# Tanveer81/ReVisionLLM

Hardware: AMD Instinct MI355X
Metric: video-segments/sec (whole node), stage-2 100-seg recursion, Vicuna-7B (higher is better)
Workload: dtype fp16

## Files before the change

### revisionllm_amd/csrc/engine.hip

```cpp
#include <string>
#include <unordered_map>
#include <vector>

#include "kernels.h"

struct Tensor {
    const void* p = nullptr;
    int dtype = 0;
    int64_t numel = 0;
};

struct AdapterLayer {
    const op16_t *w_in, *w_out, *w1, *w2;
    const float *b_in, *b_out, *b1, *b2, *ln1_w, *ln1_b, *ln2_w, *ln2_b;
};
struct LlmLayer {
    const op16_t *wqkv, *wo, *wgu, *wdown;
    const float *norm1, *norm2;
    const uint8_t *wqkv8 = nullptr, *wo8 = nullptr, *wgu8 = nullptr, *wdown8 = nullptr;
    const float *sqkv = nullptr, *so = nullptr, *sgu = nullptr, *sdown = nullptr;
    const uint8_t *wqkv8p = nullptr, *wo8p = nullptr, *wgu8p = nullptr, *wdown8p = nullptr;
    const op16_t *wqkv2 = nullptr, *wo2 = nullptr, *wgu2 = nullptr, *wdown2 = nullptr;
};

// ... 224 lines not shown
#define RV_TRY(expr)            \
    do {                        \
        int rc__ = (expr);      \
        if (rc__) return rc__;  \
    } while (0)

}

extern "C" int rv_ctx_create(const rv_config* cfg, rv_ctx** out) {
    RV_CHECK_ARG(out, "rv_ctx_create: null argument");
    if (!cfg) {
        rv_ctx* c = new rv_ctx();
        memset(&c->cfg, 0, sizeof(c->cfg));
        c->options_only = true;
        c->opt = g_default_opts;
        *out = c;
        return RV_OK;
    }
    RV_CHECK_ARG(cfg->hidden > 0 && cfg->heads > 0 && cfg->hidden % cfg->heads == 0, "rv_ctx_create: bad hidden/heads");
    RV_CHECK_ARG(cfg->hidden / cfg->heads == 128, "rv_ctx_create: LLM head dim must be 128 (got %d)", cfg->hidden / cfg->heads);
    RV_CHECK_ARG(cfg->hidden % 128 == 0 && cfg->inter % 128 == 0, "rv_ctx_create: hidden and inter must be multiples of 128");
    RV_CHECK_ARG(cfg->adapter_heads == 8 && (cfg->adapter_dim == 768 || (cfg->adapter_dim == 4096 && cfg->adapter_dim == cfg->hidden)),
                 "rv_ctx_create: the adapter is 768-d, or hidden-wide (4096) for the cross_attn ClipEncoder, with 8 heads");
    RV_CHECK_ARG(cfg->adapter_ff % 128 == 0 && cfg->adapter_layers >= 1, "rv_ctx_create: bad adapter ff/layers");
    rv_ctx* c = new rv_ctx();
    c->cfg = *cfg;
    c->opt = g_default_opts;
    *out = c;
    return RV_OK;
}

extern "C" void rv_ctx_destroy(rv_ctx* ctx) { delete ctx; }

namespace {
int* option_slot(RvOpts& o, const char* key) {
    const std::string k(key);
    if (k == "gemm_tile_variant") return &o.gemm_tile_variant;
    if (k == "gemm_cus") return &o.gemm_cus;
    if (k == "fp8_decode") return &o.fp8_decode;
    if (k == "fp8_prefill") return &o.fp8_prefill;
    if (k == "sample_variant") return &o.sample_variant;
    if (k == "gemm_arows") return &o.gemm_arows;
    if (k == "rows_fill") return &o.rows_fill;
    if (k == "rows_spread") return &o.rows_spread;
    if (k == "rows_persistent") return &o.rows_persistent;
    if (k == "rows_single") return &o.rows_single;
    if (k == "gemm_waves") return &o.gemm_waves;
    if (k == "gemm_mhalf") return &o.gemm_mhalf;
    if (k == "precision") return &o.precision;
    if (k == "lm_head_split") return &o.lm_head_split;
    if (k == "last_block_rows") return &o.last_block_rows;
    if (k == "adapter_stream16") return &o.adapter_stream16;
    if (k == "adapter_fold_t2v") return &o.adapter_fold_t2v;
    if (k == "attn_lds") return &o.attn_lds;
    if (k == "qkv_lds") return &o.qkv_lds;
    return nullptr;
}
}

unsigned int* rv_numeric_bound();

extern "C" int rv_ctx_set_option(rv_ctx* c, const char* key, int64_t value) {
    RV_CHECK_ARG(c && key, "rv_ctx_set_option: null argument");
    if (std::string(key) == "saturated") {
        RV_CHECK_ARG(value == 0, "rv_ctx_set_option: 'saturated' can only be reset to 0");
        if (unsigned int* p = rv_numeric_bound()) {
            if (hipDeviceSynchronize() != hipSuccess || hipMemset(p, 0, 16) != hipSuccess) {
                rv_set_error("rv_ctx_set_option: resetting the numeric status failed: %s", hipGetErrorString(hipGetLastError()));
                return RV_ERR_HIP;
            }
        }
        return RV_OK;
    }
    int* slot = option_slot(c->opt, key);
    RV_CHECK_ARG(slot, "rv_ctx_set_option: unknown option '%s'", key);
    const std::string k(key);
    if (k == "gemm_tile_variant") RV_CHECK_ARG(value >= 0 && value <= 6, "rv_ctx_set_option: gemm_tile_variant must be in [0, 6]");
    if (k == "gemm_waves") RV_CHECK_ARG(value == 4 || value == 8, "rv_ctx_set_option: gemm_waves must be 4 or 8");
    if (k == "gemm_cus") RV_CHECK_ARG(value >= 0 && value % 8 == 0, "rv_ctx_set_option: gemm_cus must be a non-negative multiple of 8");
    if (k == "precision") RV_CHECK_ARG(value == 0 || value == 1, "rv_ctx_set_option: precision must be 0 (bf16 operands) or 1 (parity: split operands)");
    *slot = (int)value;
    return RV_OK;
}

extern "C" int rv_ctx_get_option(const rv_ctx* c, const char* key, int64_t* value) {
    RV_CHECK_ARG(c && key && value, "rv_ctx_get_option: null argument");
    if (std::string(key) == "saturated") {
        *value = 0;
        if (unsigned int* p = rv_numeric_bound()) {
            unsigned int n = 0;
            if (hipDeviceSynchronize() != hipSuccess || hipMemcpy(&n, p, sizeof(n), hipMemcpyDeviceToHost) != hipSuccess) {
                rv_set_error("rv_ctx_get_option: reading the numeric status failed: %s", hipGetErrorString(hipGetLastError()));
                return RV_ERR_HIP;
            }
            *value = n;
        }
        return RV_OK;
    }
    const int* slot = option_slot(const_cast<rv_ctx*>(c)->opt, key);
    RV_CHECK_ARG(slot, "rv_ctx_get_option: unknown option '%s'", key);
    *value = *slot;
    return RV_OK;
}

extern "C" int rv_weights_bind(rv_ctx* c, const char* name, const void* dptr, int dtype, int64_t numel) {
    RV_CHECK_ARG(c && name && dptr && numel > 0, "rv_weights_bind: bad arguments");
// ... 11 lines not shown
    const int64_t d = c->cfg.adapter_dim, D = c->cfg.hidden;
    return rv_gemm_impl(x_bf16, d, c->proj_w, d, 1, c->proj_b, nullptr, 0, y, D, out_dtype, RV_ACT_NONE, rows, D, d, nullptr, 0, as_stream(stream));
}

extern "C" size_t rv_clip_encoder_ws_bytes(const rv_ctx* c, int32_t N, int32_t T, int32_t Nq, int32_t Lq) {
    if (!c || N <= 0 || T <= 0) return 0;
    return carve_clip(c, nullptr, 0, N, T, Nq, Lq).bytes;
}

extern "C" int rv_clip_encoder(rv_ctx* c, const void* x, const void* txt, const uint8_t* txt_mask, int32_t N, int32_t T,
                               int32_t Nq, int32_t Lq, int32_t feature, float* out, void* ws, size_t ws_bytes, void* stream) {
    RV_CHECK_ARG(c && x && out && ws, "rv_clip_encoder: null argument");
    RvOptScope scope(&c->opt);
    RV_CHECK_ARG(N > 0 && T > 0, "rv_clip_encoder: empty input N=%d T=%d", N, T);
    RV_CHECK_ARG(feature == RV_FEAT_CLS || feature == RV_FEAT_ALL, "rv_clip_encoder: feature must be CLS or ALL");
    RV_TRY(resolve_adapter(c));
    const bool text = c->cfg.adapter_text != 0;
    if (text) {
        RV_CHECK_ARG(txt && txt_mask && Nq > 0 && Lq > 0, "rv_clip_encoder: text features required (clip_adapter_text)");
        RV_CHECK_ARG(N % Nq == 0, "rv_clip_encoder: N=%d must be a multiple of Nq=%d", N, Nq);
    }
    hipStream_t st = as_stream(stream);
    const ClipWs w = carve_clip(c, ws, ws_bytes, N, T, text ? Nq : 0, text ? Lq : 0);
    if (w.bytes > ws_bytes) {
        rv_set_error("rv_clip_encoder: workspace %zu < required %zu", ws_bytes, w.bytes);
        return RV_ERR_WORKSPACE;
    }
    const int64_t d = c->cfg.adapter_dim, ff = c->cfg.adapter_ff, D = c->cfg.hidden;
    const int H = c->cfg.adapter_heads, dh = (int)(d / H);
    const float scale = 1.0f / sqrtf((float)dh);
    const int64_t R0 = (int64_t)N * T, R1 = (int64_t)N * (T + 1);

    const bool s16 = RV_OP_F16 != 0 && c->adp_proj_w != nullptr && c->opt.adapter_stream16 != 0 && (int64_t)N * T > 32;
    op16_t* xs16 = (op16_t*)w.x32;
    op16_t* ys16 = (op16_t*)w.y32;
    RV_TRY(k_copy_f32(c->cls_pos, w.pm, d, st));
    RV_TRY(k_sine_pos(w.pm + d, T, (int)d, st));

    if (text) {
        const int64_t RT = (int64_t)Nq * Lq;
        hipLaunchKernelGGL(invert_mask_kernel, dim3((unsigned)cdiv(RT, 256)), dim3(256), 0, st, txt_mask, w.pad, (int)RT);
        RV_CHECK_LAUNCH("invert_mask");
        float* v32 = w.x32;
        op16_t* vp16 = w.xp16;
        RV_TRY(k_frames_in(x, w.pm + d, s16 ? nullptr : v32, vp16, R0, T, (int)d, st));
        const op16_t* vres16 = (const op16_t*)x;
        for (size_t l = 0; l < c->t2v.size(); ++l) {
            const AdapterLayer& L = c->t2v[l];
            op16_t* q16 = w.qk16;
            RV_TRY(rv_gemm_impl(txt, d, L.w_in + d * d, d, 1, L.b_in + d, nullptr, 0, w.tk16, 2 * d, RV_OP16, RV_ACT_NONE, RT, 2 * d, d, w.sk, w.sk_bytes, st));
            const int LK = Lq <= 16 ? 16 : 32;
            const int64_t NK = (int64_t)H * LK, Rq = (int64_t)(N / Nq) * T;
            const bool fold = c->opt.adapter_fold_t2v != 0 && Lq <= 32 && dh <= 128 && NK % 64 == 0 && Rq > 32;
            if (fold) {
                float* S32 = (float*)w.qk16;
                op16_t* P16 = w.a16;
                RV_TRY(k_t2v_fold(L.w_in, L.b_in, L.w_out, w.tk16, w.tv16, 2 * d, Nq, Lq, LK, H, dh, scale, w.fa1, w.fc1, w.fa2, st));
                if (Nq > 1) {
                    RV_TRY(rv_gemm_grouped_impl(vp16, d, w.fa1, NK * d, w.fc1, NK, nullptr, 0, S32, NK, RV_F32, R0, NK, d, Rq, st));
                    RV_TRY(k_t2v_softmax(S32, w.pad, P16, R0, H, LK, Lq, Rq, st));
                    if (s16)
                        RV_TRY(rv_gemm_grouped_impl(P16, NK, w.fa2, NK * d, L.b_out, 0, (const float*)vres16, d, ys16, d, RV_OP16, R0, d, NK, Rq, st, 1));
                    else
                        RV_TRY(rv_gemm_grouped_impl(P16, NK, w.fa2, NK * d, L.b_out, 0, v32, d, w.y32, d, RV_F32, R0, d, NK, Rq, st));
                }
                for (int qi = 0; qi < Nq && Nq == 1; ++qi)
                    RV_TRY(rv_gemm_impl(vp16 + qi * Rq * d, d, w.fa1 + qi * NK * d, d, 1, w.fc1 + qi * NK, nullptr, 0, S32 + qi * Rq * NK, NK, RV_F32, RV_ACT_NONE, Rq, NK, d,
                                        w.sk, w.sk_bytes, st));
                if (Nq == 1) RV_TRY(k_t2v_softmax(S32, w.pad, P16, R0, H, LK, Lq, Rq, st));
                for (int qi = 0; qi < Nq && Nq == 1; ++qi) {
                    const int64_t r0 = qi * Rq;
                    if (s16)
                        RV_TRY(rv_gemm_impl(P16 + r0 * NK, NK, w.fa2 + qi * NK * d, NK, 1, L.b_out, (const float*)(vres16 + r0 * d), d, ys16 + r0 * d, d, RV_OP16, RV_ACT_NONE, Rq, d,
                                            NK, w.sk, w.sk_bytes, st, nullptr, 1));
                    else
                        RV_TRY(rv_gemm_impl(P16 + r0 * NK, NK, w.fa2 + qi * NK * d, NK, 1, L.b_out, v32 + r0 * d, d, w.y32 + r0 * d, d, RV_F32, RV_ACT_NONE, Rq, d, NK, w.sk,
                                            w.sk_bytes, st));
                }
            } else {
                RV_TRY(rv_gemm_impl(vp16, d, L.w_in, d, 1, L.b_in, nullptr, 0, q16, d, RV_OP16, RV_ACT_NONE, R0, d, d, w.sk, w.sk_bytes, st));
                RV_TRY(k_transpose_v(w.tv16, 2 * d, w.tvt16, Nq, Lq, w.Lqpad, H, dh, st));
                AttnArgs a{q16, d, (int64_t)T * d, w.tk16, 2 * d, (int64_t)Lq * 2 * d, dh, w.tvt16, (int64_t)d * w.Lqpad, (int64_t)dh * w.Lqpad,
                           w.Lqpad, w.a16, d, (int64_t)T * d, w.pad, N, H, dh, T, Lq, 0, 0, N / Nq, scale};
                RV_TRY(k_attention(a, st));
            }
            if (s16) {
                if (!fold)
                    RV_TRY(rv_gemm_impl(w.a16, d, L.w_out, d, 1, L.b_out, (const float*)vres16, d, ys16, d, RV_OP16, RV_ACT_NONE, R0, d, d, w.sk, w.sk_bytes, st, nullptr, 1));
                RV_TRY(k_layernorm(nullptr, L.ln1_w, L.ln1_b, nullptr, w.x16, nullptr, nullptr, 0, R0, (int)d, st, 0, ys16));
                RV_TRY(rv_gemm_impl(w.x16, d, L.w1, d, 1, L.b1, nullptr, 0, w.h16, ff, RV_OP16, RV_ACT_RELU, R0, ff, d, w.sk, w.sk_bytes, st));
                RV_TRY(rv_gemm_impl(w.h16, ff, L.w2, ff, 1, L.b2, (const float*)ys16, d, ys16, d, RV_OP16, RV_ACT_NONE, R0, d, ff, w.sk, w.sk_bytes, st, nullptr, 1));
                if (l + 1 < c->t2v.size()) {
                    RV_TRY(k_layernorm(nullptr, L.ln2_w, L.ln2_b, nullptr, xs16, vp16, w.pm + d, T, R0, (int)d, st, 0, ys16));
                    vres16 = xs16;
                } else {
                    RV_TRY(k_layernorm(nullptr, L.ln2_w, L.ln2_b, nullptr, w.x16, w.xp16, w.pm + d, T, R0, (int)d, st, T, ys16));
                    RV_TRY(k_cls_rows(c->cls_token, w.pm, nullptr, w.x16, w.xp16, N, T, (int)d, st));
                }
                continue;
            }
            if (!fold)
                RV_TRY(rv_gemm_impl(w.a16, d, L.w_out, d, 1, L.b_out, v32, d, w.y32, d, RV_F32, RV_ACT_NONE, R0, d, d, w.sk, w.sk_bytes, st));
            RV_TRY(k_layernorm(w.y32, L.ln1_w, L.ln1_b, nullptr, w.x16, nullptr, nullptr, 0, R0, (int)d, st));
            RV_TRY(rv_gemm_impl(w.x16, d, L.w1, d, 1, L.b1, nullptr, 0, w.h16, ff, RV_OP16, RV_ACT_RELU, R0, ff, d, w.sk, w.sk_bytes, st));
            RV_TRY(rv_gemm_impl(w.h16, ff, L.w2, ff, 1, L.b2, w.y32, d, w.y32, d, RV_F32, RV_ACT_NONE, R0, d, ff, w.sk, w.sk_bytes, st));
            if (l + 1 < c->t2v.size()) {
                RV_TRY(k_layernorm(w.y32, L.ln2_w, L.ln2_b, v32, nullptr, vp16, w.pm + d, T, R0, (int)d, st));
            } else {
                RV_TRY(k_layernorm(w.y32, L.ln2_w, L.ln2_b, w.x32, w.x16, w.xp16, w.pm + d, T, R0, (int)d, st, T));
                RV_TRY(k_cls_rows(c->cls_token, w.pm, w.x32, w.x16, w.xp16, N, T, (int)d, st));
            }
        }
    } else {
        RV_TRY(k_build_x(x, nullptr, c->cls_token, w.pm, s16 ? nullptr : w.x32, w.x16, w.xp16, N, T, (int)d, st));
    }

    for (size_t l = 0; l < c->enc.size(); ++l) {
        const AdapterLayer& L = c->enc[l];
        if (feature == RV_FEAT_CLS && l + 1 == c->enc.size() && N > 16 && T >= 3) {
            const int64_t sx = (int64_t)(T + 1) * d;
            op16_t* kk16 = w.qk16;
            op16_t* qc16 = w.h16;
            float* y0 = w.y32;
            float* y1 = w.y32 + (int64_t)N * d;
            float* y2 = w.y32 + (int64_t)2 * N * d;
            RV_TRY(rv_gemm_impl(w.xp16, d, L.w_in + d * d, d, 1, L.b_in + d, nullptr, 0, kk16, d, RV_OP16, RV_ACT_NONE, R1, d, d, w.sk, w.sk_bytes, st));
            RV_TRY(rv_gemm_impl(w.xp16, sx, L.w_in, d, 1, L.b_in, nullptr, 0, qc16, d, RV_OP16, RV_ACT_NONE, N, d, d, w.sk, w.sk_bytes, st, nullptr, 0, 1));
            RV_TRY(rv_gemm_impl(w.x16, d, L.w_in + 2 * d * d, d, 1, L.b_in + 2 * d, nullptr, 0, w.vv16, d, RV_OP16, RV_ACT_NONE, R1, d, d, w.sk, w.sk_bytes, st));
            RV_TRY(k_transpose_v(w.vv16, d, w.vt16, N, T + 1, w.Lpad, H, dh, st));
            AttnArgs a{qc16, d, d, kk16, d, (int64_t)(T + 1) * d, dh, w.vt16, (int64_t)d * w.Lpad, (int64_t)dh * w.Lpad, w.Lpad, w.a16, d, d,
                       nullptr, N, H, dh, 1, T + 1, 0, 0, 1, scale, 1};
            RV_TRY(k_attention(a, st));
            const float* cls_res = w.x32;
            int64_t cls_ld = sx;
            if (s16) {
                float* y3 = w.y32 + (int64_t)3 * N * d;
                RV_TRY(k_rows_to_f32(w.x16, sx, y3, N, (int)d, st));
                cls_res = y3;
                cls_ld = d;
            }
            RV_TRY(rv_gemm_impl(w.a16, d, L.w_out, d, 1, L.b_out, cls_res, cls_ld, y0, d, RV_F32, RV_ACT_NONE, N, d, d, w.sk, w.sk_bytes, st, nullptr, 0, 1));
            RV_TRY(k_layernorm(y0, L.ln1_w, L.ln1_b, y1, w.x16, nullptr, nullptr, 0, N, (int)d, st, 0, nullptr, s16 ? 3 : 0));
// ... 533 lines not shown
```

### revisionllm_amd/csrc/kernels.h

```cpp
#pragma once
#include "common.h"

struct RvOpts {
    int gemm_tile_variant = 2;
    int gemm_cus = 0;
    int fp8_decode = 1;
    int fp8_prefill = 1;
    int sample_variant = 1;
    int gemm_arows = 1;
    int gemm_waves = 8;
    int gemm_mhalf = 2;
    int rows_single = 1;
    int rows_persistent = 1;
    int rows_spread = 0;
    int rows_fill = 240;
    int lm_head_split = 1;
    int last_block_rows = 1;
    int adapter_stream16 = 1;
    int adapter_fold_t2v = 1;
    int attn_lds = 1;
    int qkv_lds = 1;
    int precision = 0;
};
extern const RvOpts g_default_opts;
const RvOpts& rv_cur_opts();
struct RvOptScope {
    const RvOpts* prev;
    explicit RvOptScope(const RvOpts* o);
    ~RvOptScope();
};
const RvOpts* rv_ctx_opts(const rv_ctx* c);

struct GemvNorm {
    const float* in_sumsq = nullptr;
    int in_nblk = 0;
    float inv_d = 0.f, eps = 0.f;
    void* xw_out = nullptr;
    const float* w_next = nullptr;
    float* out_sumsq = nullptr;
    const float* w_scale = nullptr;
    int x_packed = 0;
    int out_packed = 0;
    float* planes = nullptr;
    int* arrive = nullptr;
};
__host__ __device__ __forceinline__ int64_t rv_xp_index(int r, int k, int mbp) {
    return ((((int64_t)(k >> 5) * mbp + (r >> 4)) * 64 + (r & 15) + 16 * ((k >> 3) & 3)) * 8) + (k & 7);
}
constexpr int RV_ROWS_COUNTERS = 2048;
constexpr int RV_ROWS_MAX = 144;
constexpr int RV_XP_MAX_BLOCKS = 9;
__host__ __device__ __forceinline__ int rv_xp_blocks(int64_t rows) { return rows <= 32 ? 2 : rows <= 64 ? 4 : rows <= 80 ? 5 : rows <= 128 ? 8 : 9; }

constexpr int RV_MAX_PREFILL_GROUPS = 8;
__host__ __device__ __forceinline__ int64_t rv_vt_index(int d, int pos) { return ((int64_t)(pos >> 3) * 128 + d) * 8 + (pos & 7); }
struct alignas(32) QkvGroup {
    int base, B, S, P0, row, pad_[3];
};
struct QkvRope {
    const float* cs = nullptr;
    void* q16 = nullptr;
    void* kc = nullptr;
    void* vtc = nullptr;
    int B = 0, S = 0, P0 = 0, pos0 = 0, cs_pos0 = 0, H = 0, Smax = 0;
    const int* row_pos = nullptr;
    int G = 1, Mg = 0;
    int grow[RV_MAX_PREFILL_GROUPS] = {0, 0, 0, 0, 0, 0, 0, 0};
    int q_ld = 0, q_lo = 0;
    int ng = 0;
    const QkvGroup* gt = nullptr;
};
static __device__ __forceinline__ QkvGroup qkv_rope_group(const QkvRope& q, int& m) {
// ... 91 lines not shown
}
static __device__ __forceinline__ void qkv_rope_store(const QkvRope& q, int m, int n, f32x4 v) {
    qkv_rope_store(q, m, n, v, qkv_rope_coeffs(q, m, n));
}

int gemm_qkv_rope(const void* A, int64_t lda, const void* Wp, int64_t M, int64_t D, const QkvRope& r, const GemvNorm* norm,
                  void* ws, size_t ws_bytes, hipStream_t st, int w_layout = 1, int64_t Kdim = 0);

int rv_gemm_impl(const void* A, int64_t lda, const void* W, int64_t ldw, int w_layout, const float* bias,
                 const float* residual, int64_t ldr, void* C, int64_t ldc, int out_dtype, int act, int64_t M, int64_t N,
                 int64_t K, void* ws, size_t ws_bytes, hipStream_t st, const GemvNorm* norm = nullptr, int res16 = 0, int no_stream = 0);
struct GemmGroups {
    int rows = 0, tiles = 0;
    int64_t w_stride = 0, bias_stride = 0;
};
int rv_gemm_grouped_impl(const void* A, int64_t lda, const void* Wp, int64_t w_stride, const float* bias, int64_t bias_stride, const float* residual, int64_t ldr, void* C,
                         int64_t ldc, int out_dtype, int64_t M, int64_t N, int64_t K, int64_t rows_per_group, hipStream_t st, int res16 = 0);
int gemv_blocks(int act, int64_t N);
int gemm_rows(const op16_t* X, const op16_t* W, const float* bias, const float* res, int64_t ldr, void* C, int64_t ldc, int out_dtype, int act,
              int M, int N, int K, hipStream_t st, const GemvNorm& nrm, const QkvRope* qr, int w_layout = 1);
size_t gemm_rows_ws_bytes();
bool gemm_arows_supported(int w_layout, int act, int64_t M, int64_t N, int64_t K);
int gemm_arows_launch(const void* A, int64_t lda, const void* Wp, const float* bias, const float* res, int64_t ldr, void* C, int64_t ldc,
                      int out_dtype, int act, int64_t M, int64_t N, int64_t K, hipStream_t st);
bool gemm_pp_supported(int w_layout, int64_t M, int64_t N, int64_t K);
bool gemm_pp_sk_supported(int w_layout, int64_t M, int64_t N, int64_t K);
int gemm_pp_sk_plan(int64_t M, int64_t N, int64_t K, bool gated);
bool gemm_pp_sk_profitable(int64_t M, int64_t N, int64_t K);
bool gemm_pp_dp_profitable(int64_t M, int64_t N, int64_t K);
int gemm_pp_dp_plan(int64_t M, int64_t N, int64_t K, bool gated);
size_t gemm_pp_ws_bytes();
bool gemm_pp_fp8_supported(int64_t M, int64_t N, int64_t K, bool gated, bool rope);
int gemm_pp_fp8(const void* A8, int64_t lda, const float* sa, const void* W8p, const float* sw, const float* res, int64_t ldr, void* C,
                int64_t ldc, int out_dtype, int act, int64_t M, int64_t N, int64_t K, const QkvRope* r, void* ws, hipStream_t st);
int gemm_pp_launch(const void* A, int64_t lda, const void* Wp, const float* bias, const float* res, int64_t ldr, void* C,
                   int64_t ldc, int out_dtype, int act, int64_t M, int64_t N, int64_t K, void* ws, hipStream_t st);
int gemm_pp_qkv_rope(const void* A, int64_t lda, const void* Wp, int64_t M, int64_t N, int64_t K, const QkvRope& r, void* ws,
                     hipStream_t st);
int k_layernorm(const float* x, const float* w, const float* b, float* y32, void* y16, void* yp16, const float* pos,
                int64_t period, int64_t rows, int d, hipStream_t st, int64_t gap = 0, const void* x_op16 = nullptr, int rnd = 0);
int k_rmsnorm_quant(const float* x, int64_t x_row_stride, const float* w, void* q8, float* scale, int64_t rows, int d, float eps,
                    hipStream_t st);
int k_quant_rows_fp8(const void* x16, int64_t ldx, void* q8, int64_t ldq, float* scale, int64_t rows, int K, hipStream_t st);
int k_rmsnorm(const float* x, int64_t x_row_stride, const float* w, void* y16, int64_t rows, int d, float eps, hipStream_t st,
              int out_packed = 0, const int* row_idx = nullptr);
int k_rmsnorm_split(const float* x, int64_t x_row_stride, const float* w, void* y16, int64_t rows, int d, float eps, hipStream_t st, int out_packed = 0,
                    const int* row_idx = nullptr);
int k_split_bf16(const float* x, int64_t ldx, void* y16, int64_t rows, int n, hipStream_t st);
int k_qkv_rope_split(const float* qkv32, int64_t ld, const QkvRope& qr, int64_t M, int64_t D, hipStream_t st);
int k_gather_last_rows(const void* a16, const float* h, const int* idx, int64_t rows, int Mg, int P0, int B, int S, void* a_out, float* h_out, int D, hipStream_t st);
int k_t2v_fold(const void* wq_p, const float* bq, const void* wo_p, const void* tk16, const void* tv16, int64_t ld, int Nq, int Lq, int LK, int H, int dh, float scale,
               void* A1p, float* c1, void* A2p, hipStream_t st);
int k_t2v_softmax(const float* S, const uint8_t* pad, void* P16, int64_t rows, int H, int LK, int Lq, int64_t rows_per_query, hipStream_t st);
int k_sine_pos(float* pos, int T, int d, hipStream_t st);
int k_frames_in(const void* x16, const float* pos, float* v32, void* vp16, int64_t rows, int T, int d, hipStream_t st);
int k_build_x(const void* src16, const float* src32, const float* cls, const float* pm, float* x32, void* x16, void* xp16,
              int64_t N, int T, int d, hipStream_t st);
int k_copy_f32(const float* src, float* dst, int64_t n, hipStream_t st);
int k_rows_to_f32(const void* src16, int64_t ld, float* dst, int64_t rows, int d, hipStream_t st);
int k_cls_rows(const float* cls, const float* pm, float* x32, void* x16, void* xp16, int64_t N, int T, int d, hipStream_t st);
int k_transpose_v(const void* v, int64_t ld, void* vt, int64_t Nb, int L, int Lpad, int H, int dh, hipStream_t st);
int k_rope_table(float* cs, int S, int pos0, int dh, float theta, hipStream_t st);
int k_rope_table_rows(float* cs, const int* row_pos, int rows, int dh, float theta, hipStream_t st);
int k_splice_embed(const int32_t* map, const void* embed, const float* video, float* h, int64_t rows, int D, hipStream_t st);

struct AttnArgs {
    const void* q; int64_t q_rs, q_bs;
    const void* k; int64_t k_rs, k_bs, k_hs;
    const void* vt; int64_t vt_bs, vt_hs, vt_ds;
    void* out; int64_t o_rs, o_bs;
    const uint8_t* key_pad;
    int B, H, dh, Lq, Lk, causal, q_pos0, kv_div;
    float scale;
    int no_split = 0;
    const int* row_pos = nullptr;
    int out_packed = 0;
    int64_t vt_ks = 8;
    int64_t out_lo = 0;
    int64_t q_lo = 0;
    const int* row_share = nullptr;
};
int k_attention(const AttnArgs& a, hipStream_t st);
struct AttnGroups {
    int G = 1;
    int64_t q_off[RV_MAX_PREFILL_GROUPS] = {0, 0, 0, 0, 0, 0, 0, 0};
    int64_t o_off[RV_MAX_PREFILL_GROUPS] = {0, 0, 0, 0, 0, 0, 0, 0};
    int64_t kv_off[RV_MAX_PREFILL_GROUPS] = {0, 0, 0, 0, 0, 0, 0, 0};
};
int k_attention_pair(const AttnArgs& a, const AttnArgs& b, hipStream_t st, const AttnGroups* groups = nullptr);
int k_attention_groups(const AttnArgs& a, hipStream_t st, const AttnGroups& groups);
struct AttnMixed {
    int G = 0, problems = 0;
    int first[RV_MAX_PREFILL_GROUPS] = {};
    QkvGroup gt[RV_MAX_PREFILL_GROUPS] = {};
};
int k_attention_mixed(const AttnArgs& a, const AttnMixed& mx, hipStream_t st);
int k_mixed_tables(const AttnMixed& mx, QkvGroup* gt, int* last_rows, hipStream_t st);
```

### revisionllm_amd/csrc/rowops.hip

```cpp
#include "common.h"
#include "kernels.h"

namespace {

template <int NV>
__global__ __launch_bounds__(256) void layernorm_kernel(const float* __restrict__ x, const float* __restrict__ w,
                                                        const float* __restrict__ b, float* __restrict__ y32,
                                                        op16_t* __restrict__ y16, op16_t* __restrict__ yp16,
                                                        const float* __restrict__ pos, int64_t period, int64_t rows, int64_t gap,
                                                        const op16_t* __restrict__ x16in, int rnd) {
    constexpr int D = NV * 256;
    const int lane = threadIdx.x & 63;
    const int64_t row = (int64_t)blockIdx.x * 4 + (threadIdx.x >> 6);
    if (row >= rows) return;
    const float* xr = x + row * D;
    const int64_t orow = gap > 0 ? row + row / gap + 1 : row;
    f32x4 v[NV];
    float s = 0.f;
#pragma unroll
    for (int i = 0; i < NV; ++i) {
        v[i] = x16in ? op16x4_to_f32(*(const u32x2*)(x16in + row * D + i * 256 + lane * 4)) : *(const f32x4*)(xr + i * 256 + lane * 4);
        if (rnd & 1) v[i] = op16x4_to_f32(pack_op16x4(f32x4{v[i][0], v[i][1], v[i][2], v[i][3]}));
        s += v[i][0] + v[i][1] + v[i][2] + v[i][3];
    }
// ... 360 lines not shown
                    const f32x4 kk = *(const f32x4*)&rr[j][t];
#pragma unroll
                    for (int e = 0; e < 4; ++e) acc += kk[e] * w[t + e];
                }
                const int hj = h * LK + j;
                if (which) A2p[(int64_t)q * NK * d + rv_wp_index(k, hj, NK)] = f32_to_op16(acc);
                else A1p[(int64_t)q * NK * d + rv_wp_index(hj, k, d)] = f32_to_op16(acc * mul);
            }
        }
        if (blockIdx.x == 0 && threadIdx.x < 64) {
            for (int j = 0; j < LK; ++j) {
                float c = 0.f;
                for (int t = threadIdx.x; t < DH; t += 64) c += rr[j][t] * bq[h * DH + t];
                c = wave_sum(c);
                if (threadIdx.x == 0) c1[(int64_t)q * NK + h * LK + j] = c * scale;
            }
        }
    }
}

template <int LK>
__global__ __launch_bounds__(256) void t2v_softmax_kernel(const float* __restrict__ S, const uint8_t* __restrict__ pad, op16_t* __restrict__ P, int64_t rows, int H, int Lq,
                                                          int64_t rows_per_query) {
    const int64_t i = (int64_t)blockIdx.x * 256 + threadIdx.x;
    if (i >= rows * H) return;
    const int64_t r = i / H;
    const uint8_t* pq = pad + (r / rows_per_query) * Lq;
    unsigned valid = 0u;
    for (int j = 0; j < Lq; ++j) valid |= (pq[j] == 0 ? 1u : 0u) << j;
    const f32x4* s4 = (const f32x4*)(S + i * LK);
    f32x4 v[LK / 4];
    float mx = -INFINITY;
#pragma unroll
    for (int c = 0; c < LK / 4; ++c) {
        v[c] = s4[c];
#pragma unroll
        for (int e = 0; e < 4; ++e) {
            if (!((valid >> (c * 4 + e)) & 1u)) v[c][e] = -INFINITY;
            mx = fmaxf(mx, v[c][e]);
        }
    }
    float z = 0.f;
#pragma unroll
    for (int c = 0; c < LK / 4; ++c)
#pragma unroll
        for (int e = 0; e < 4; ++e) {
            v[c][e] = mx == -INFINITY ? 0.f : __expf(v[c][e] - mx);
            z += v[c][e];
        }
    const float iz = z > 0.f ? 1.0f / z : 0.f;
    u32x2* p2 = (u32x2*)(P + i * LK);
#pragma unroll
    for (int c = 0; c < LK / 4; ++c) p2[c] = pack_op16x4(f32x4{v[c][0] * iz, v[c][1] * iz, v[c][2] * iz, v[c][3] * iz});
}

__global__ void rope_table_kernel(float2* __restrict__ cs, int S, int pos0, int dh, float theta) {
    const int i = blockIdx.x * blockDim.x + threadIdx.x;
    const int half = dh / 2;
    if (i >= S * half) return;
    const int s = i / half, j = i % half;
    const float inv = 1.0f / powf(theta, (float)(2 * j) / (float)dh);
    const float ang = (float)(pos0 + s) * inv;
    cs[i] = make_float2(cosf(ang), sinf(ang));
}

__global__ void rope_table_rows_kernel(float2* __restrict__ cs, const int* __restrict__ row_pos, int rows, int dh, float theta) {
    const int i = blockIdx.x * blockDim.x + threadIdx.x;
    const int half = dh / 2;
    if (i >= rows * half) return;
    const int s = i / half, j = i % half;
    const int pos = row_pos[s] > 0 ? row_pos[s] : 0;
    const float inv = 1.0f / powf(theta, (float)(2 * j) / (float)dh);
    const float ang = (float)pos * inv;
    cs[i] = make_float2(cosf(ang), sinf(ang));
}

__global__ __launch_bounds__(256) void splice_embed_kernel(const int32_t* __restrict__ map, const op16_t* __restrict__ embed,
                                                           const float* __restrict__ video, float* __restrict__ h, int D) {
    const int64_t r = blockIdx.x;
    const int src = map[r];
    float* o = h + r * D;
    if (src >= 0) {
        const op16_t* e = embed + (int64_t)src * D;
        for (int c = threadIdx.x * 4; c < D; c += 1024) {
            const u32x2 raw = *(const u32x2*)(e + c);
            *(f32x4*)(o + c) = op16x4_to_f32(raw);
        }
    } else {
        const float* v = video + (int64_t)(-(src + 1)) * D;
        for (int c = threadIdx.x * 4; c < D; c += 1024) *(f32x4*)(o + c) = *(const f32x4*)(v + c);
    }
}

}

int k_layernorm(const float* x, const float* w, const float* b, float* y32, void* y16, void* yp16, const float* pos,
                int64_t period, int64_t rows, int d, hipStream_t st, int64_t gap, const void* x_op16, int rnd) {
    RV_CHECK_ARG((x || x_op16) && w && b && rows >= 0, "layernorm: bad arguments");
    RV_CHECK_ARG(!yp16 || (pos && period > 0), "layernorm: y_pos needs pos table and period");
    if (rows == 0) return RV_OK;
    const unsigned blocks = (unsigned)cdiv(rows, 4);
    if (d == 768)
        hipLaunchKernelGGL(layernorm_kernel<3>, dim3(blocks), dim3(256), 0, st, x, w, b, y32, (op16_t*)y16, (op16_t*)yp16, pos, period, rows, gap, (const op16_t*)x_op16, rnd);
    else if (d == 4096)
        hipLaunchKernelGGL(layernorm_kernel<16>, dim3(blocks), dim3(256), 0, st, x, w, b, y32, (op16_t*)y16, (op16_t*)yp16, pos, period, rows, gap, (const op16_t*)x_op16, rnd);
    else if (d == 1024)
// ... 115 lines not shown
    if (dh == 96)
        hipLaunchKernelGGL(transpose_v_kernel<96>, grid, dim3(256), 0, st, (const op16_t*)v, ld, (op16_t*)vt, L, Lpad, H);
    else if (dh == 128)
        hipLaunchKernelGGL(transpose_v_kernel<128>, grid, dim3(256), 0, st, (const op16_t*)v, ld, (op16_t*)vt, L, Lpad, H);
    else if (dh == 512)
        hipLaunchKernelGGL(transpose_v_kernel<512>, dim3(grid.x, grid.y * 4, grid.z), dim3(256), 0, st, (const op16_t*)v, ld, (op16_t*)vt, L, Lpad, H);
    else {
        rv_set_error("transpose_v: head dim %d unsupported", dh);
        return RV_ERR_ARG;
    }
    RV_CHECK_LAUNCH("transpose_v");
    return RV_OK;
}

int k_gather_last_rows(const void* a16, const float* h, const int* idx, int64_t rows, int Mg, int P0, int B, int S, void* a_out, float* h_out, int D, hipStream_t st) {
    RV_CHECK_ARG(a16 && h && a_out && h_out && rows > 0 && D % 4 == 0, "gather_last_rows: bad arguments");
    hipLaunchKernelGGL(gather_last_rows_kernel, dim3((unsigned)rows), dim3(256), 0, st, (const op16_t*)a16, h, idx, Mg, P0, B, S, (op16_t*)a_out, h_out, D);
    RV_CHECK_LAUNCH("gather_last_rows");
    return RV_OK;
}

int k_t2v_fold(const void* wq_p, const float* bq, const void* wo_p, const void* tk16, const void* tv16, int64_t ld, int Nq, int Lq, int LK, int H, int dh, float scale,
               void* A1p, float* c1, void* A2p, hipStream_t st) {
    const int d = H * dh;
    RV_CHECK_ARG(wq_p && bq && wo_p && tk16 && tv16 && A1p && c1 && A2p && ld >= d && Nq > 0 && Lq > 0 && Lq <= LK && (LK == 16 || LK == 32) && dh <= 128 && d % 32 == 0,
                 "t2v_fold: bad arguments");
#define RV_FOLD_REG(DH_, LK_)                                                                                                                                  \
    hipLaunchKernelGGL((t2v_fold_reg_kernel<DH_, LK_>), dim3((unsigned)(2 * cdiv(d, 256)), (unsigned)H, (unsigned)cdiv(Nq, qpw)), dim3(256), 0, st, (const op16_t*)wq_p, bq, \
                       (const op16_t*)wo_p, (const op16_t*)tk16, (const op16_t*)tv16, ld, Lq, H, d, scale, (op16_t*)A1p, c1, (op16_t*)A2p, Nq, qpw)
    const bool reg = Nq >= 3;
    const int qpw = (int)cdiv((int64_t)Nq * 2 * cdiv(d, 256) * H, 1024);
    if (reg && dh == 96 && LK == 16) RV_FOLD_REG(96, 16);
    else if (reg && dh == 96 && LK == 32) RV_FOLD_REG(96, 32);
    else if (reg && dh == 64 && LK == 16) RV_FOLD_REG(64, 16);
    else if (reg && dh == 64 && LK == 32) RV_FOLD_REG(64, 32);
    else
        hipLaunchKernelGGL(t2v_fold_kernel, dim3((unsigned)cdiv(d, 256), (unsigned)(H * LK), (unsigned)Nq), dim3(256), 0, st, (const op16_t*)wq_p, bq, (const op16_t*)wo_p,
                           (const op16_t*)tk16, (const op16_t*)tv16, ld, Lq, LK, H, dh, d, scale, (op16_t*)A1p, c1, (op16_t*)A2p);
#undef RV_FOLD_REG
    RV_CHECK_LAUNCH("t2v_fold");
    return RV_OK;
}

int k_t2v_softmax(const float* S, const uint8_t* pad, void* P16, int64_t rows, int H, int LK, int Lq, int64_t rows_per_query, hipStream_t st) {
    RV_CHECK_ARG(S && pad && P16 && rows > 0 && (LK == 16 || LK == 32) && Lq <= LK && rows_per_query > 0, "t2v_softmax: bad arguments");
    if (LK == 16)
        hipLaunchKernelGGL(t2v_softmax_kernel<16>, dim3((unsigned)cdiv(rows * H, 256)), dim3(256), 0, st, S, pad, (op16_t*)P16, rows, H, Lq, rows_per_query);
    else
        hipLaunchKernelGGL(t2v_softmax_kernel<32>, dim3((unsigned)cdiv(rows * H, 256)), dim3(256), 0, st, S, pad, (op16_t*)P16, rows, H, Lq, rows_per_query);
    RV_CHECK_LAUNCH("t2v_softmax");
    return RV_OK;
}

int k_rope_table(float* cs, int S, int pos0, int dh, float theta, hipStream_t st) {
    hipLaunchKernelGGL(rope_table_kernel, dim3((unsigned)cdiv((int64_t)S * (dh / 2), 256)), dim3(256), 0, st, (float2*)cs, S, pos0, dh, theta);
    RV_CHECK_LAUNCH("rope_table");
    return RV_OK;
}

int k_rope_table_rows(float* cs, const int* row_pos, int rows, int dh, float theta, hipStream_t st) {
    hipLaunchKernelGGL(rope_table_rows_kernel, dim3((unsigned)cdiv((int64_t)rows * (dh / 2), 256)), dim3(256), 0, st, (float2*)cs, row_pos, rows, dh, theta);
    RV_CHECK_LAUNCH("rope_table_rows");
    return RV_OK;
}

int k_splice_embed(const int32_t* map, const void* embed, const float* video, float* h, int64_t rows, int D, hipStream_t st) {
    hipLaunchKernelGGL(splice_embed_kernel, dim3((unsigned)rows), dim3(256), 0, st, map, (const op16_t*)embed, video, h, D);
    RV_CHECK_LAUNCH("splice_embed");
    return RV_OK;
}

extern "C" int rv_layernorm(const float* x, const float* w, const float* b, float* y_f32, void* y_bf16, void* y_pos_bf16,
                            const float* pos, int64_t period, int64_t rows, int32_t d, void* stream) {
    return k_layernorm(x, w, b, y_f32, y_bf16, y_pos_bf16, pos, period, rows, d, as_stream(stream));
}
extern "C" int rv_rmsnorm(const float* x, const float* w, void* y_bf16, int64_t rows, int32_t d, float eps, void* stream) {
    return k_rmsnorm(x, d, w, y_bf16, rows, d, eps, as_stream(stream));
}
extern "C" int rv_rmsnorm_quant_fp8(const float* x, const float* w, void* q8, float* scale, int64_t rows, int32_t d, float eps, void* stream) {
    RV_CHECK_ARG(x && w && q8 && scale, "rv_rmsnorm_quant_fp8: null argument");
    return k_rmsnorm_quant(x, d, w, q8, scale, rows, d, eps, as_stream(stream));
}
extern "C" int rv_sine_pos(float* pos, int32_t T, int32_t d, void* stream) { return k_sine_pos(pos, T, d, as_stream(stream)); }
```

### revisionllm_amd/hip.py

```python
import ctypes as C
import os

import torch

_HERE = os.path.dirname(os.path.abspath(__file__))
LIB_PATHS = {"f16": os.environ.get("REVISION_HIP_LIB") or os.path.join(_HERE, "librevision_hip.so"),
             "bf16": os.environ.get("REVISION_HIP_LIB_BF16") or os.path.join(_HERE, "librevision_hip_bf16.so")}
LIB_PATH = LIB_PATHS["f16"]
OP_DTYPES = {"f16": torch.float16, "bf16": torch.bfloat16}

RV_F32, RV_BF16, RV_I32, RV_I64, RV_U8, RV_F16 = 0, 1, 2, 3, 4, 5
RV_ACT_NONE, RV_ACT_RELU, RV_ACT_SILU_MUL, RV_ACT_QUICK_GELU = 0, 1, 2, 3
RV_FEAT_CLS, RV_FEAT_ALL = 0, 2
TOPK_CAP = 64

_DT = {torch.float32: RV_F32, torch.bfloat16: RV_BF16, torch.float16: RV_F16, torch.int32: RV_I32, torch.int64: RV_I64, torch.uint8: RV_U8}


class RvConfig(C.Structure):
    _fields_ = [("hidden", C.c_int32), ("inter", C.c_int32), ("layers", C.c_int32), ("heads", C.c_int32),
                ("vocab", C.c_int32), ("rms_eps", C.c_float), ("rope_theta", C.c_float), ("adapter_dim", C.c_int32),
                ("adapter_heads", C.c_int32), ("adapter_ff", C.c_int32), ("adapter_layers", C.c_int32),
                ("adapter_text", C.c_int32)]

# ... 147 lines not shown
            raise HipLibraryError(
                f"{path} not found: build it with `python -m revisionllm_amd.build` (hipcc, gfx950). "
                "revisionllm_amd has no CPU fallback.")
        try:
            h = C.CDLL(path)
        except OSError as e:
            raise HipLibraryError(f"cannot load {path}: {e}") from e
        for name, (res, args) in SIGNATURES.items():
            fn = getattr(h, name)
            fn.restype, fn.argtypes = res, args
        if h.rv_operand_dtype() != _DT[OP_DTYPES[f]]:
            raise HipLibraryError(f"{path} is not the {f} build of the library (rv_operand_dtype() = {h.rv_operand_dtype()})")
        _libs[f] = h
    return h


_numeric = {}


def numeric_status(f=None, device=None):
    f = flavour_of(f)
    dev = torch.device("cuda", torch.cuda.current_device()) if device is None else torch.device(device)
    if dev.index is None:
        dev = torch.device("cuda", torch.cuda.current_device())
    key = (f, dev.index)
    t = _numeric.get(key)
    if t is None:
        t = torch.zeros(4, dtype=torch.int32, device=dev)
        with torch.cuda.device(dev):
            torch.cuda.synchronize(dev)
            check(lib(f).rv_numeric_status_bind(C.c_void_p(t.data_ptr())), "rv_numeric_status_bind")
        _numeric[key] = t
    return t


def last_error():
    buf = C.create_string_buffer(512)
    msgs = []
    for h in _libs.values():
        h.rv_last_error(buf, 512)
        if buf.value:
            msgs.append(buf.value.decode())
    return " | ".join(msgs)


def check(rc, what):
    if rc != 0:
        msgs = last_error().split(" | ")
        name = what.split("(")[0]
        mine = [m for m in msgs if name in m]
        raise HipLibraryError(f"{what} failed (status {rc}): {' | '.join(mine or msgs)}")


OPTION_KEYS = ("gemm_tile_variant", "gemm_cus", "gemm_arows", "fp8_decode", "fp8_prefill", "sample_variant", "rows_fill", "rows_spread", "rows_persistent", "rows_single", "gemm_waves", "gemm_mhalf", "precision", "lm_head_split", "last_block_rows", "adapter_stream16", "adapter_fold_t2v", "attn_lds", "qkv_lds")


class Options:

    def __init__(self, flavour=None, **kw):
        self.flavour = flavour_of(flavour)
        self.lib = lib(self.flavour)
        self._ctx = C.c_void_p()
        check(self.lib.rv_ctx_create(None, C.byref(self._ctx)), "rv_ctx_create(options)")
        for k, v in kw.items():
            self.set(k, v)

    def set(self, key, value):
        check(self.lib.rv_ctx_set_option(self._ctx, key.encode(), int(value)), f"rv_ctx_set_option({key})")
        return self

    def get(self, key):
        v = _i64()
        check(self.lib.rv_ctx_get_option(self._ctx, key.encode(), C.byref(v)), f"rv_ctx_get_option({key})")
        return int(v.value)

    def __del__(self):
        try:
            if self._ctx and self._ctx.value:
                self.lib.rv_ctx_destroy(self._ctx)
                self._ctx = C.c_void_p()
        except Exception:
            pass


def ctx_ptr(ctx, f=None):
    if ctx is None:
        return None
    if f is not None and ctx.flavour != flavour_of(f):
        raise HipLibraryError(f"a {ctx.flavour} context was passed to a {flavour_of(f)} call")
    return ctx._ctx


def ptr(t):
    if t is None:
        return None
    if not t.is_cuda:
        raise HipLibraryError("librevision_hip needs device tensors (got a CPU tensor); there is no CPU path")
    return C.c_void_p(t.data_ptr())


def stream():
    return C.c_void_p(torch.cuda.current_stream().cuda_stream)


def dtype_code(t):
    return _DT[t.dtype]
```

Measured before the change: 6493.

## Fuse folded text-to-video attention, residual and layernorm into one row kernel

Adds a per-16-row wavefront kernel for the folded t2v adapter attention. It computes scores against the folded query-key matrix, the masked softmax, the projection through the folded value-output matrix, bias and residual add, and the first layernorm, all in registers. This replaces two grouped GEMMs, a softmax kernel and a layernorm launch, and avoids writing and rereading the fp32 score and fp16 probability intermediates. It is restricted to the 16-bit stream path with d=768 and H=8, and puts a heavy register load on the kernel, which may limit occupancy.

```diff
diff --git a/revisionllm_amd/csrc/engine.hip b/revisionllm_amd/csrc/engine.hip
--- a/revisionllm_amd/csrc/engine.hip
+++ b/revisionllm_amd/csrc/engine.hip
@@ -300,6 +300,7 @@
     if (k == "last_block_rows") return &o.last_block_rows;
     if (k == "adapter_stream16") return &o.adapter_stream16;
     if (k == "adapter_fold_t2v") return &o.adapter_fold_t2v;
+    if (k == "adapter_t2v_rows") return &o.adapter_t2v_rows;
     if (k == "attn_lds") return &o.attn_lds;
     if (k == "qkv_lds") return &o.qkv_lds;
     return nullptr;
@@ -417,11 +418,13 @@
             const int LK = Lq <= 16 ? 16 : 32;
             const int64_t NK = (int64_t)H * LK, Rq = (int64_t)(N / Nq) * T;
             const bool fold = c->opt.adapter_fold_t2v != 0 && Lq <= 32 && dh <= 128 && NK % 64 == 0 && Rq > 32;
+            const bool rows1 = fold && s16 && c->opt.adapter_t2v_rows != 0 && d == 768 && H == 8;
             if (fold) {
                 float* S32 = (float*)w.qk16;
                 op16_t* P16 = w.a16;
                 RV_TRY(k_t2v_fold(L.w_in, L.b_in, L.w_out, w.tk16, w.tv16, 2 * d, Nq, Lq, LK, H, dh, scale, w.fa1, w.fc1, w.fa2, st));
-                if (Nq > 1) {
+                if (rows1) RV_TRY(k_t2v_rows(vp16, w.fa1, w.fc1, w.fa2, L.b_out, vres16, ys16, L.ln1_w, L.ln1_b, w.x16, w.pad, Nq, Lq, LK, H, (int)d, Rq, st));
+                if (!rows1 && Nq > 1) {
                     RV_TRY(rv_gemm_grouped_impl(vp16, d, w.fa1, NK * d, w.fc1, NK, nullptr, 0, S32, NK, RV_F32, R0, NK, d, Rq, st));
                     RV_TRY(k_t2v_softmax(S32, w.pad, P16, R0, H, LK, Lq, Rq, st));
                     if (s16)
@@ -429,11 +432,11 @@
                     else
                         RV_TRY(rv_gemm_grouped_impl(P16, NK, w.fa2, NK * d, L.b_out, 0, v32, d, w.y32, d, RV_F32, R0, d, NK, Rq, st));
                 }
-                for (int qi = 0; qi < Nq && Nq == 1; ++qi)
+                for (int qi = 0; qi < Nq && Nq == 1 && !rows1; ++qi)
                     RV_TRY(rv_gemm_impl(vp16 + qi * Rq * d, d, w.fa1 + qi * NK * d, d, 1, w.fc1 + qi * NK, nullptr, 0, S32 + qi * Rq * NK, NK, RV_F32, RV_ACT_NONE, Rq, NK, d,
                                         w.sk, w.sk_bytes, st));
-                if (Nq == 1) RV_TRY(k_t2v_softmax(S32, w.pad, P16, R0, H, LK, Lq, Rq, st));
-                for (int qi = 0; qi < Nq && Nq == 1; ++qi) {
+                if (Nq == 1 && !rows1) RV_TRY(k_t2v_softmax(S32, w.pad, P16, R0, H, LK, Lq, Rq, st));
+                for (int qi = 0; qi < Nq && Nq == 1 && !rows1; ++qi) {
                     const int64_t r0 = qi * Rq;
                     if (s16)
                         RV_TRY(rv_gemm_impl(P16 + r0 * NK, NK, w.fa2 + qi * NK * d, NK, 1, L.b_out, (const float*)(vres16 + r0 * d), d, ys16 + r0 * d, d, RV_OP16, RV_ACT_NONE, Rq, d,
@@ -452,7 +455,8 @@
             if (s16) {
                 if (!fold)
                     RV_TRY(rv_gemm_impl(w.a16, d, L.w_out, d, 1, L.b_out, (const float*)vres16, d, ys16, d, RV_OP16, RV_ACT_NONE, R0, d, d, w.sk, w.sk_bytes, st, nullptr, 1));
-                RV_TRY(k_layernorm(nullptr, L.ln1_w, L.ln1_b, nullptr, w.x16, nullptr, nullptr, 0, R0, (int)d, st, 0, ys16));
+                if (!rows1)
+                    RV_TRY(k_layernorm(nullptr, L.ln1_w, L.ln1_b, nullptr, w.x16, nullptr, nullptr, 0, R0, (int)d, st, 0, ys16));
                 RV_TRY(rv_gemm_impl(w.x16, d, L.w1, d, 1, L.b1, nullptr, 0, w.h16, ff, RV_OP16, RV_ACT_RELU, R0, ff, d, w.sk, w.sk_bytes, st));
                 RV_TRY(rv_gemm_impl(w.h16, ff, L.w2, ff, 1, L.b2, (const float*)ys16, d, ys16, d, RV_OP16, RV_ACT_NONE, R0, d, ff, w.sk, w.sk_bytes, st, nullptr, 1));
                 if (l + 1 < c->t2v.size()) {
diff --git a/revisionllm_amd/csrc/kernels.h b/revisionllm_amd/csrc/kernels.h
--- a/revisionllm_amd/csrc/kernels.h
+++ b/revisionllm_amd/csrc/kernels.h
@@ -18,6 +18,7 @@
     int last_block_rows = 1;
     int adapter_stream16 = 1;
     int adapter_fold_t2v = 1;
+    int adapter_t2v_rows = 1;
     int attn_lds = 1;
     int qkv_lds = 1;
     int precision = 0;
@@ -215,6 +216,8 @@
 int k_t2v_fold(const void* wq_p, const float* bq, const void* wo_p, const void* tk16, const void* tv16, int64_t ld, int Nq, int Lq, int LK, int H, int dh, float scale,
                void* A1p, float* c1, void* A2p, hipStream_t st);
 int k_t2v_softmax(const float* S, const uint8_t* pad, void* P16, int64_t rows, int H, int LK, int Lq, int64_t rows_per_query, hipStream_t st);
+int k_t2v_rows(const void* xp16, const void* A1p, const float* c1, const void* A2p, const float* b_out, const void* res16, void* ys16, const float* ln_w, const float* ln_b,
+               void* x16, const uint8_t* pad, int Nq, int Lq, int LK, int H, int d, int64_t rows_per_query, hipStream_t st);
 int k_sine_pos(float* pos, int T, int d, hipStream_t st);
 int k_frames_in(const void* x16, const float* pos, float* v32, void* vp16, int64_t rows, int T, int d, hipStream_t st);
 int k_build_x(const void* src16, const float* src32, const float* cls, const float* pm, float* x32, void* x16, void* xp16,
diff --git a/revisionllm_amd/csrc/rowops.hip b/revisionllm_amd/csrc/rowops.hip
--- a/revisionllm_amd/csrc/rowops.hip
+++ b/revisionllm_amd/csrc/rowops.hip
@@ -436,6 +436,153 @@
     u32x2* p2 = (u32x2*)(P + i * LK);
 #pragma unroll
     for (int c = 0; c < LK / 4; ++c) p2[c] = pack_op16x4(f32x4{v[c][0] * iz, v[c][1] * iz, v[c][2] * iz, v[c][3] * iz});
+}
+
+template <int LK>
+__global__ __launch_bounds__(256, 2) void t2v_rows_kernel(const op16_t* __restrict__ xp, const op16_t* __restrict__ A1p, const float* __restrict__ c1,
+                                                       const op16_t* __restrict__ A2p, const float* __restrict__ bo, const op16_t* __restrict__ res, op16_t* __restrict__ ys,
+                                                       const float* __restrict__ lnw, const float* __restrict__ lnb, op16_t* __restrict__ x16,
+                                                       const uint8_t* __restrict__ pad, int Lq, int64_t Rq, int Nq) {
+    constexpr int D = 768, H = 8, NK = H * LK, NT = NK / 16, KS1 = D / 32, KS2 = NK / 32, NP = D / 32;
+    const int lane = threadIdx.x & 63, m = lane & 15, g = lane >> 4;
+    const int64_t tpq = (Rq + 15) >> 4;
+    const int64_t tile = (int64_t)blockIdx.x * 4 + (threadIdx.x >> 6);
+    if (tile >= tpq * Nq) return;
+    const int q = (int)(tile / tpq);
+    const int64_t rl = (tile - q * tpq) * 16 + m;
+    const bool live = rl < Rq;
+    const int64_t row = (int64_t)q * Rq + (live ? rl : Rq - 1);
+    unsigned valid = 0u;
+    for (int j = 0; j < Lq; ++j) valid |= (pad[(int64_t)q * Lq + j] == 0 ? 1u : 0u) << j;
+
+    f32x4 s[NT];
+#pragma unroll
+    for (int t = 0; t < NT; ++t) s[t] = f32x4{0.f, 0.f, 0.f, 0.f};
+    const op16_t* xr = xp + row * D + g * 8;
+    const op16_t* a1 = A1p + (int64_t)q * NK * D + lane * 8;
+    op16x8 xb[KS1];
+#pragma unroll
+    for (int ks = 0; ks < KS1; ++ks) xb[ks] = *(const op16x8*)(xr + ks * 32);
+#pragma unroll
+    for (int ks = 0; ks < KS1; ++ks) {
+#pragma unroll
+        for (int t = 0; t < NT; ++t) s[t] = rv_mfma16(*(const op16x8*)(a1 + (t * KS1 + ks) * 512), xb[ks], s[t]);
+    }
+
+    union { op16x8 v; uint32_t u[4]; } P[KS2];
+    const float* cq = c1 + (int64_t)q * NK + g * 4;
+    constexpr int TPH = LK / 16;
+#pragma unroll
+    for (int h = 0; h < H; ++h) {
+        float v[TPH][4];
+        float mx = -INFINITY;
+#pragma unroll
+        for (int u = 0; u < TPH; ++u) {
+            const int t = h * TPH + u;
+            const f32x4 cc = *(const f32x4*)(cq + t * 16);
+#pragma unroll
+            for (int i = 0; i < 4; ++i) {
+                v[u][i] = ((valid >> (u * 16 + g * 4 + i)) & 1u) ? s[t][i] + cc[i] : -INFINITY;
+                mx = fmaxf(mx, v[u][i]);
+            }
+        }
+        mx = fmaxf(mx, __shfl_xor(mx, 16, 64));
+        mx = fmaxf(mx, __shfl_xor(mx, 32, 64));
+        float z = 0.f;
+#pragma unroll
+        for (int u = 0; u < TPH; ++u)
+#pragma unroll
+            for (int i = 0; i < 4; ++i) {
+                v[u][i] = mx == -INFINITY ? 0.f : __expf(v[u][i] - mx);
+                z += v[u][i];
+            }
+        z += __shfl_xor(z, 16, 64);
+        z += __shfl_xor(z, 32, 64);
+        const float iz = z > 0.f ? 1.0f / z : 0.f;
+#pragma unroll
+        for (int u = 0; u < TPH; ++u) {
+            const int t = h * TPH + u;
+            P[t >> 1].u[2 * (t & 1)] = pack_op16x2_bounded(v[u][0] * iz, v[u][1] * iz);
+            P[t >> 1].u[2 * (t & 1) + 1] = pack_op16x2_bounded(v[u][2] * iz, v[u][3] * iz);
+        }
+    }
+
+    const op16_t* a2 = A2p + (int64_t)q * NK * D + ((m >> 3) * KS2 * 64 + 8 * ((m >> 2) & 1) + (m & 3) + 16 * (g >> 1)) * 8 + 4 * (g & 1);
+    const int64_t o0 = row * D + g * 8;
+    uint32_t yk[NP][4];
+    float sum = 0.f;
+    uint32_t sat = 0;
+    constexpr int RA = 6;
+    u32x4 rq[NP];
+    auto res_load = [&](int p) { rq[p] = *(const u32x4*)(res + o0 + p * 32); };
+#pragma unroll
+    for (int p = 0; p < RA; ++p) res_load(p);
+#pragma unroll
+    for (int p = 0; p < NP; ++p) {
+        if (p + RA < NP) res_load(p + RA);
+        f32x4 acc[2] = {f32x4{0.f, 0.f, 0.f, 0.f}, f32x4{0.f, 0.f, 0.f, 0.f}};
+#pragma unroll
+        for (int ks = 0; ks < KS2; ++ks)
+#pragma unroll
+            for (int sb = 0; sb < 2; ++sb) {
+                const op16_t* b = a2 + (p * 2 * KS2 + ks) * 512 + sb * 32;
+                union { op16x8 v; u32x2 h[2]; } af;
+                af.h[0] = *(const u32x2*)b;
+                af.h[1] = *(const u32x2*)(b + 256);
+                acc[sb] = rv_mfma16(af.v, P[ks].v, acc[sb]);
+            }
+        const int n = p * 32 + g * 8;
+        const f32x4 b0 = *(const f32x4*)(bo + n), b1 = *(const f32x4*)(bo + n + 4);
+        const f32x4 r0 = op16x4_to_f32(u32x2{rq[p][0], rq[p][1]}), r1 = op16x4_to_f32(u32x2{rq[p][2], rq[p][3]});
+        f32x4 y0, y1;
+#pragma unroll
+        for (int i = 0; i < 4; ++i) {
+            y0[i] = acc[0][i] + b0[i] + r0[i];
+            y1[i] = acc[1][i] + b1[i] + r1[i];
+        }
+        yk[p][0] = pack_op16x2_m(y0[0], y0[1], sat);
+        yk[p][1] = pack_op16x2_m(y0[2], y0[3], sat);
+        yk[p][2] = pack_op16x2_m(y1[0], y1[1], sat);
+        yk[p][3] = pack_op16x2_m(y1[2], y1[3], sat);
+        if (live) *(u32x4*)(ys + o0 + p * 32) = u32x4{yk[p][0], yk[p][1], yk[p][2], yk[p][3]};
+        const f32x4 a = op16x4_to_f32(u32x2{yk[p][0], yk[p][1]}), c = op16x4_to_f32(u32x2{yk[p][2], yk[p][3]});
+        sum += a[0] + a[1] + a[2] + a[3] + c[0] + c[1] + c[2] + c[3];
+    }
+    {
+        rv_note_saturation(live ? sat : 0u);
+        sum += __shfl_xor(sum, 16, 64);
+        sum += __shfl_xor(sum, 32, 64);
+        const float mean = sum * (1.0f / D);
+        float qq = 0.f;
+#pragma unroll
+        for (int p = 0; p < NP; ++p) {
+            const f32x4 a = op16x4_to_f32(u32x2{yk[p][0], yk[p][1]}), c = op16x4_to_f32(u32x2{yk[p][2], yk[p][3]});
+#pragma unroll
+            for (int i = 0; i < 4; ++i) {
+                const float da = a[i] - mean, dc = c[i] - mean;
+                qq += da * da;
+                qq += dc * dc;
+            }
+        }
+        qq += __shfl_xor(qq, 16, 64);
+        qq += __shfl_xor(qq, 32, 64);
+        const float rstd = rsqrtf(qq * (1.0f / D) + 1e-5f);
+        if (!live) return;
+#pragma unroll
+        for (int p = 0; p < NP; ++p) {
+            const int n = p * 32 + g * 8;
+            const f32x4 a = op16x4_to_f32(u32x2{yk[p][0], yk[p][1]}), c = op16x4_to_f32(u32x2{yk[p][2], yk[p][3]});
+            const f32x4 w0 = *(const f32x4*)(lnw + n), w1 = *(const f32x4*)(lnw + n + 4), e0 = *(const f32x4*)(lnb + n), e1 = *(const f32x4*)(lnb + n + 4);
+            f32x4 ya, yc;
+#pragma unroll
+            for (int i = 0; i < 4; ++i) {
+                ya[i] = (a[i] - mean) * rstd * w0[i] + e0[i];
+                yc[i] = (c[i] - mean) * rstd * w1[i] + e1[i];
+            }
+            const u32x2 pa = pack_op16x4(ya), pc = pack_op16x4(yc);
+            *(u32x4*)(x16 + o0 + p * 32) = u32x4{pa[0], pa[1], pc[0], pc[1]};
+        }
+    }
 }
 
 __global__ void rope_table_kernel(float2* __restrict__ cs, int S, int pos0, int dh, float theta) {
@@ -657,6 +804,25 @@
     return RV_OK;
 }
 
+int k_t2v_rows(const void* xp16, const void* A1p, const float* c1, const void* A2p, const float* b_out, const void* res16, void* ys16, const float* ln_w, const float* ln_b,
+               void* x16, const uint8_t* pad, int Nq, int Lq, int LK, int H, int d, int64_t rows_per_query, hipStream_t st) {
+    RV_CHECK_ARG(xp16 && A1p && c1 && A2p && b_out && res16 && ys16 && ln_w && ln_b && x16 && pad && Nq > 0 && Lq > 0 && Lq <= LK && (LK == 16 || LK == 32) && H == 8 &&
+                     d == 768 && rows_per_query > 0,
+                 "t2v_rows: bad arguments");
+    RV_CHECK_ARG((((uintptr_t)xp16 | (uintptr_t)A1p | (uintptr_t)c1 | (uintptr_t)A2p | (uintptr_t)b_out | (uintptr_t)res16 | (uintptr_t)ys16 | (uintptr_t)ln_w | (uintptr_t)ln_b |
+                   (uintptr_t)x16) & 15) == 0,
+                 "t2v_rows: every buffer must be 16-byte aligned");
+    const unsigned blocks = (unsigned)cdiv(cdiv(rows_per_query, 16) * Nq, 4);
+#define RV_T2V_ROWS(LK_)                                                                                                                                               \
+    hipLaunchKernelGGL((t2v_rows_kernel<LK_>), dim3(blocks), dim3(256), 0, st, (const op16_t*)xp16, (const op16_t*)A1p, c1, (const op16_t*)A2p, b_out, (const op16_t*)res16, \
+                       (op16_t*)ys16, ln_w, ln_b, (op16_t*)x16, pad, Lq, rows_per_query, Nq)
+    if (LK == 16) RV_T2V_ROWS(16);
+    else RV_T2V_ROWS(32);
+#undef RV_T2V_ROWS
+    RV_CHECK_LAUNCH("t2v_rows");
+    return RV_OK;
+}
+
 int k_rope_table(float* cs, int S, int pos0, int dh, float theta, hipStream_t st) {
     hipLaunchKernelGGL(rope_table_kernel, dim3((unsigned)cdiv((int64_t)S * (dh / 2), 256)), dim3(256), 0, st, (float2*)cs, S, pos0, dh, theta);
     RV_CHECK_LAUNCH("rope_table");
diff --git a/revisionllm_amd/hip.py b/revisionllm_amd/hip.py
--- a/revisionllm_amd/hip.py
+++ b/revisionllm_amd/hip.py
@@ -223,7 +223,7 @@
         raise HipLibraryError(f"{what} failed (status {rc}): {' | '.join(mine or msgs)}")
 
 
-OPTION_KEYS = ("gemm_tile_variant", "gemm_cus", "gemm_arows", "fp8_decode", "fp8_prefill", "sample_variant", "rows_fill", "rows_spread", "rows_persistent", "rows_single", "gemm_waves", "gemm_mhalf", "precision", "lm_head_split", "last_block_rows", "adapter_stream16", "adapter_fold_t2v", "attn_lds", "qkv_lds")
+OPTION_KEYS = ("gemm_tile_variant", "gemm_cus", "gemm_arows", "fp8_decode", "fp8_prefill", "sample_variant", "rows_fill", "rows_spread", "rows_persistent", "rows_single", "gemm_waves", "gemm_mhalf", "precision", "lm_head_split", "last_block_rows", "adapter_stream16", "adapter_fold_t2v", "adapter_t2v_rows", "attn_lds", "qkv_lds")
 
 
 class Options:
```

Measured after the change: 6487. About the same (-0.1%).
